# liangyuwang/Tiny-DeepSpeed

Measured on AMD Instinct MI355X. Metric: tokens/sec (whole node) GPT-2 ZeRO-2, higher is better.
Workload: dtype bf16; 1 GPU; model=gpt2-medium, global_batch=32, seq_len=1024, parallelism=zero2-dp1

## Files before the change

csrc/bind.cpp:

```cpp
#include <torch/extension.h>
#include <ATen/cuda/CUDAContext.h>

#include <hip/hip_runtime_api.h>

#include <array>
#include <cstring>
#include <vector>

extern "C" {
hipError_t tdsa_ln_fwd(const void*, const void*, void*, const void*,
                       const void*, void*, float*, float*, int, int, float,
                       int, hipStream_t);
int tdsa_ln_bwd_dx_stripes(int M);
hipError_t tdsa_ln_bwd_dx(const void*, const void*, const void*, const void*,
                          const float*, const float*, void*, float*, float*,
                          int, int, int, hipStream_t);
hipError_t tdsa_ln_bwd_dwdb(const float*, const float*, float*, float*, int,
                            int, hipStream_t);
hipError_t tdsa_gelu_fwd(const void*, void*, long long, int, hipStream_t);
hipError_t tdsa_gelu_bwd(const void*, const void*, void*, long long, int,
                         hipStream_t);
hipError_t tdsa_column_sum(const void*, float*, void*, int, int, int,
                           hipStream_t);
hipError_t tdsa_embedding_fwd(const void*, const long long*, void*, long long,
                              int, int, hipStream_t);
hipError_t tdsa_embedding_bwd(const void*, const long long*, const long long*,
                              float*, float*, long long, int, long long, int,
                              hipStream_t);
hipError_t tdsa_ce_fwd(const void*, const long long*, float*, float*, int*,
                       long long, int, long long, int, hipStream_t);
hipError_t tdsa_ce_bwd(const void*, const long long*, const float*, void*,
                       long long, int, float, long long, int, hipStream_t);
hipError_t tdsa_adamw_step(void*, const void*, float*, float*, float*, float*,
                           int, int, float, float, float, float, float,
                           long long, long long, int, int, hipStream_t);
hipError_t tdsa_adamw_multi(const void*, long long, int, int, float, float,
                            float, float, float, long long, hipStream_t);
int tdsa_adamw_desc_size();
int tdsa_adamw_chunkref_size();
int tdsa_sgd_desc_size();
hipError_t tdsa_sgd_multi(const void*, long long, int, int, float, float,
                          float, float, int, int, int, hipStream_t);
hipError_t tdsa_sgd_step(void*, const void*, float*, float*, int, int, float,
                         float, float, float, int, int, int, long long, int,
                         int, hipStream_t);
hipError_t tdsa_attn_fwd(const void*, const void*, const void*, void*, float*,
                         long long, long long, int, float, const long long*,
                         const long long*, float, unsigned long long,
                         hipStream_t);
hipError_t tdsa_attn_bwd(const void*, const void*, const void*, const void*,
                         const float*, const void*, void*, void*, void*, float*,
                         long long, long long, int, float, const long long*,
                         const long long*, const long long*, float,
                         unsigned long long, hipStream_t);
int tdsa_gemm_tn_splits(long long M, int N, int K);
hipError_t tdsa_gemm_tn(const void*, const void*, float*, long long, int, int,
                        hipStream_t);
hipError_t tdsa_dbg_mfma(const void*, const void*, float*, int, hipStream_t);
hipError_t tdsa_dbg_mfma32(const void*, const void*, float*, hipStream_t);
hipError_t tdsa_dbg_stage(const void*, void*, int, hipStream_t);
hipError_t tdsa_dbg_tr16(const void*, float*, hipStream_t);
}

namespace {

void check_hip(hipError_t err, const char* what) {
  TORCH_CHECK(err == hipSuccess, what, ": ", hipGetErrorString(err));
}

int dtype_flag(const at::Tensor& t) {
  if (t.scalar_type() == at::kBFloat16) return 1;
  if (t.scalar_type() == at::kFloat) return 0;
  TORCH_CHECK(false, "expected float32 or bfloat16, got ", t.scalar_type());
  return -1;
}

hipStream_t cur_stream() {
  return (hipStream_t)at::cuda::getCurrentCUDAStream().stream();
}

#define CHECK_IN(t)                                                     \
  TORCH_CHECK((t).is_cuda(), #t " must be on GPU");                     \
  TORCH_CHECK((t).is_contiguous(), #t " must be contiguous")

std::vector<at::Tensor> layernorm_fwd(at::Tensor x, at::Tensor w, at::Tensor b,
                                      double eps,
                                      c10::optional<at::Tensor> res) {
  CHECK_IN(x); CHECK_IN(w); CHECK_IN(b);
  const int N = x.size(-1);
  const long long M = x.numel() / N;
  auto y = at::empty_like(x);
  auto f32 = x.options().dtype(at::kFloat);
  auto mean = at::empty({M}, f32);
  auto rstd = at::empty({M}, f32);
  at::Tensor h;
  void* res_p = nullptr;
  void* h_p = nullptr;
  if (res.has_value()) {
    CHECK_IN((*res));
    h = at::empty_like(x);
    res_p = res->data_ptr();
    h_p = h.data_ptr();
  }
  check_hip(tdsa_ln_fwd(x.data_ptr(), res_p, h_p, w.data_ptr(), b.data_ptr(),
                        y.data_ptr(), mean.data_ptr<float>(),
                        rstd.data_ptr<float>(), (int)M, N, (float)eps,
                        dtype_flag(x), cur_stream()),
            "layernorm_fwd");
  auto row_sizes = x.sizes().vec();
  row_sizes.pop_back();
  if (res.has_value())
    return {y, mean.view(row_sizes), rstd.view(row_sizes), h};
  return {y, mean.view(row_sizes), rstd.view(row_sizes)};
}

std::vector<at::Tensor> layernorm_bwd_dx(at::Tensor dy, at::Tensor x,
                                         at::Tensor w, at::Tensor mean,
                                         at::Tensor rstd, int64_t n_stripes,
                                         c10::optional<at::Tensor> dh) {
  CHECK_IN(dy); CHECK_IN(x); CHECK_IN(w);
  (void)n_stripes;
  const int N = x.size(-1);
  const long long M = x.numel() / N;
  const int G = tdsa_ln_bwd_dx_stripes((int)M);
  auto dx = at::empty_like(x);
  auto f32 = x.options().dtype(at::kFloat);
  auto pdw = at::empty({G, N}, f32);
  auto pdb = at::empty({G, N}, f32);
  auto meanc = mean.contiguous();
  auto rstdc = rstd.contiguous();
  at::Tensor dhc;
  void* dh_p = nullptr;
  if (dh.has_value()) {
    dhc = dh->contiguous();
    dh_p = dhc.data_ptr();
  }
  check_hip(tdsa_ln_bwd_dx(dy.data_ptr(), dh_p, x.data_ptr(), w.data_ptr(),
                           meanc.data_ptr<float>(), rstdc.data_ptr<float>(),
                           dx.data_ptr(), pdw.data_ptr<float>(),
                           pdb.data_ptr<float>(), (int)M, N, dtype_flag(x),
                           cur_stream()),
            "layernorm_bwd_dx");
  return {dx, pdw, pdb};
}

std::vector<at::Tensor> layernorm_bwd_dwdb(at::Tensor pdw, at::Tensor pdb) {
  CHECK_IN(pdw); CHECK_IN(pdb);
  const int G = pdw.size(0);
  const int N = pdw.size(1);
  auto dw = at::empty({N}, pdw.options());
  auto db = at::empty({N}, pdb.options());
  check_hip(tdsa_ln_bwd_dwdb(pdw.data_ptr<float>(), pdb.data_ptr<float>(),
                             dw.data_ptr<float>(), db.data_ptr<float>(), G, N,
                             cur_stream()),
            "layernorm_bwd_dwdb");
  return {dw, db};
}

at::Tensor gelu_fwd(at::Tensor x) {
  CHECK_IN(x);
  auto y = at::empty_like(x);
  check_hip(tdsa_gelu_fwd(x.data_ptr(), y.data_ptr(), x.numel(), dtype_flag(x),
                          cur_stream()),
            "gelu_fwd");
  return y;
}

at::Tensor gelu_bwd(at::Tensor dy, at::Tensor x) {
  CHECK_IN(dy); CHECK_IN(x);
  auto dx = at::empty_like(x);
  check_hip(tdsa_gelu_bwd(dy.data_ptr(), x.data_ptr(), dx.data_ptr(), x.numel(),
                          dtype_flag(x), cur_stream()),
            "gelu_bwd");
  return dx;
}

at::Tensor column_sum(at::Tensor dy) {
  CHECK_IN(dy);
  TORCH_CHECK(dy.dim() == 2, "column_sum expects 2-D input");
  const int M = dy.size(0);
  const int N = dy.size(1);
  auto out32 = at::zeros({N}, dy.options().dtype(at::kFloat));
  auto out = at::empty({N}, dy.options());
  check_hip(tdsa_column_sum(dy.data_ptr(), out32.data_ptr<float>(),
                            out.data_ptr(), M, N, dtype_flag(dy), cur_stream()),
            "column_sum");
  return out;
}

at::Tensor embedding_fwd(at::Tensor weight, at::Tensor idx) {
  CHECK_IN(weight); CHECK_IN(idx);
  TORCH_CHECK(idx.scalar_type() == at::kLong, "idx must be int64");
  const long long R = idx.numel();
  const int D = weight.size(1);
  auto out = at::empty({R, (long long)D}, weight.options());
  check_hip(tdsa_embedding_fwd(weight.data_ptr(), (const long long*)idx.data_ptr<int64_t>(),
                               out.data_ptr(), R, D, dtype_flag(weight),
                               cur_stream()),
            "embedding_fwd");
  return out;
}

at::Tensor embedding_bwd(at::Tensor dy, at::Tensor idx, int64_t num_embeddings,
                         int64_t padding_idx) {
  CHECK_IN(dy); CHECK_IN(idx);
  TORCH_CHECK(idx.scalar_type() == at::kLong, "idx must be int64");
  const long long R = idx.numel();
  const int D = dy.size(-1);
  auto dw32 = at::zeros({num_embeddings, (long long)D},
                        dy.options().dtype(at::kFloat));
  auto sorted = at::sort(idx.reshape({-1}), true, 0,
                         false);
  auto sidx = std::get<0>(sorted).contiguous();
  auto perm = std::get<1>(sorted).contiguous();
  auto part = at::empty({R, (long long)D}, dy.options().dtype(at::kFloat));
  check_hip(tdsa_embedding_bwd(dy.data_ptr(), (const long long*)sidx.data_ptr<int64_t>(),
                               (const long long*)perm.data_ptr<int64_t>(),
                               dw32.data_ptr<float>(), part.data_ptr<float>(),
                               R, D, padding_idx, dtype_flag(dy),
                               cur_stream()),
            "embedding_bwd");
  return dw32;
}

std::vector<at::Tensor> cross_entropy_fwd(at::Tensor logits, at::Tensor targets,
                                          int64_t ignore_index) {
  CHECK_IN(logits); CHECK_IN(targets);
  TORCH_CHECK(logits.dim() == 2, "logits must be 2-D");
  TORCH_CHECK(targets.scalar_type() == at::kLong, "targets must be int64");
  const long long R = logits.size(0);
  const int V = logits.size(1);
  auto f32 = logits.options().dtype(at::kFloat);
  auto lse = at::empty({R}, f32);
  auto row_loss = at::empty({R}, f32);
  auto n_valid32 = at::zeros({}, logits.options().dtype(at::kInt));
  check_hip(tdsa_ce_fwd(logits.data_ptr(), (const long long*)targets.data_ptr<int64_t>(),
                        lse.data_ptr<float>(), row_loss.data_ptr<float>(),
                        n_valid32.data_ptr<int>(), R, V, ignore_index,
                        dtype_flag(logits), cur_stream()),
            "cross_entropy_fwd");
  return {row_loss.sum(), lse, n_valid32.to(at::kLong)};
}

at::Tensor cross_entropy_bwd(at::Tensor logits, at::Tensor targets,
                             at::Tensor lse, double dloss, int64_t n_valid,
                             int64_t ignore_index,
                             c10::optional<at::Tensor> out) {
  CHECK_IN(logits); CHECK_IN(targets); CHECK_IN(lse);
  const long long R = logits.size(0);
  const int V = logits.size(1);
  at::Tensor dlogits;
  if (out.has_value()) {
    dlogits = *out;
    CHECK_IN(dlogits);
    TORCH_CHECK(dlogits.sizes() == logits.sizes()
                && dlogits.scalar_type() == logits.scalar_type(),
                "cross_entropy_bwd: out must match logits");
  } else {
    dlogits = at::empty_like(logits);
  }
  const float scale = (float)(dloss / (double)std::max<int64_t>(n_valid, 1));
  check_hip(tdsa_ce_bwd(logits.data_ptr(), (const long long*)targets.data_ptr<int64_t>(),
                        lse.data_ptr<float>(), dlogits.data_ptr(), R, V, scale,
                        ignore_index, dtype_flag(logits), cur_stream()),
            "cross_entropy_bwd");
  return dlogits;
}

void adamw_step(at::Tensor param, at::Tensor grad, at::Tensor m, at::Tensor v,
                at::Tensor master, at::Tensor vmax, bool has_master,
                bool amsgrad, double lr, double b1, double b2, double eps,
                double wd, int64_t step) {
  CHECK_IN(param); CHECK_IN(grad); CHECK_IN(m); CHECK_IN(v);
  check_hip(tdsa_adamw_step(param.data_ptr(), grad.data_ptr(),
                            m.data_ptr<float>(), v.data_ptr<float>(),
                            has_master ? master.data_ptr<float>() : nullptr,
                            amsgrad ? vmax.data_ptr<float>() : nullptr,
                            has_master, amsgrad, (float)lr, (float)b1,
                            (float)b2, (float)eps, (float)wd, step,
                            param.numel(), dtype_flag(param), dtype_flag(grad),
                            cur_stream()),
            "adamw_step");
}

void adamw_step_multi(std::vector<at::Tensor> params,
                      std::vector<at::Tensor> grads,
                      std::vector<at::Tensor> ms, std::vector<at::Tensor> vs,
                      std::vector<c10::optional<at::Tensor>> masters,
                      double lr, double b1, double b2, double eps, double wd,
                      int64_t step) {
  const size_t n = params.size();
  TORCH_CHECK(grads.size() == n && ms.size() == n && vs.size() == n &&
              masters.size() == n, "length mismatch");
  if (n == 0) return;
  struct Desc {
    void* p; const void* g; float* m; float* v; float* master;
    long long numel; int param_bf16; int grad_bf16;
  };
  struct CRef { int tensor; int chunk; };
  TORCH_CHECK((int)sizeof(Desc) == tdsa_adamw_desc_size());
  TORCH_CHECK((int)sizeof(CRef) == tdsa_adamw_chunkref_size());
  const int chunk_elems = 1 << 16;
  std::vector<Desc> descs(n);
  std::vector<CRef> chunks;
  chunks.reserve(1024);
  for (size_t i = 0; i < n; ++i) {
    auto& p = params[i];
    auto& g = grads[i];
    Desc d;
// ... 77 lines not shown
  check_hip(tdsa_sgd_step(param.data_ptr(), grad.data_ptr(),
                          has_buf ? buf.data_ptr<float>() : nullptr,
                          has_master ? master.data_ptr<float>() : nullptr,
                          has_buf, has_master, (float)lr, (float)momentum,
                          (float)dampening, (float)wd, nesterov, maximize,
                          first_step, param.numel(), dtype_flag(param),
                          dtype_flag(grad), cur_stream()),
            "sgd_step");
}

at::Tensor gemm_tn(at::Tensor dy2, at::Tensor x2) {
  CHECK_IN(dy2); CHECK_IN(x2);
  TORCH_CHECK(dy2.dim() == 2 && x2.dim() == 2, "gemm_tn expects 2-D inputs");
  TORCH_CHECK(dy2.scalar_type() == at::kBFloat16
              && x2.scalar_type() == at::kBFloat16, "gemm_tn is bf16-only");
  TORCH_CHECK(dy2.size(0) == x2.size(0), "reduction dims differ");
  const long long M = dy2.size(0);
  const int N = dy2.size(1);
  const int K = x2.size(1);
  const int splits = tdsa_gemm_tn_splits(M, N, K);
  TORCH_CHECK(splits > 0, "gemm_tn: unsupported shape (need M%64==0, "
              "N%128==0, K%128==0), got ", M, "x", N, "/", K);
  auto f32 = dy2.options().dtype(at::kFloat);
  auto dw32 = at::empty({(long long)splits, (long long)N, (long long)K}, f32);
  check_hip(tdsa_gemm_tn(dy2.data_ptr(), x2.data_ptr(),
                         dw32.data_ptr<float>(), M, N, K, cur_stream()),
            "gemm_tn");
  return (splits > 1 ? dw32.sum(0) : dw32.select(0, 0)).to(at::kBFloat16);
}

static void check_attn_tensor(const at::Tensor& t, const char* name) {
  TORCH_CHECK(t.is_cuda(), name, " must be on GPU");
  TORCH_CHECK(t.dim() == 4 && t.size(3) == 64, name,
              ": attention kernel requires (B,H,T,64)");
  TORCH_CHECK(t.scalar_type() == at::kBFloat16, name, " must be bf16");
  TORCH_CHECK(t.stride(3) == 1, name, " last dim must be contiguous");
}

static std::array<long long, 3> strides3(const at::Tensor& t) {
  return {(long long)t.stride(0), (long long)t.stride(1),
          (long long)t.stride(2)};
}

std::vector<at::Tensor> attention_fwd(at::Tensor q, at::Tensor k, at::Tensor v,
                                      double scale,
                                      c10::optional<at::Tensor> out,
                                      double dropout_p, int64_t seed) {
  check_attn_tensor(q, "q");
  check_attn_tensor(k, "k");
  check_attn_tensor(v, "v");
  TORCH_CHECK(q.strides() == k.strides() && q.strides() == v.strides(),
              "q/k/v must share strides");
  TORCH_CHECK(q.size(2) % 64 == 0, "attention kernel requires T %% 64 == 0");
  const long long B = q.size(0), H = q.size(1);
  const int T = q.size(2);
  at::Tensor o = out.has_value() ? *out : at::empty_like(q);
  check_attn_tensor(o, "o");
  auto lse = at::empty({B, H, (long long)T}, q.options().dtype(at::kFloat));
  auto sq = strides3(q);
  auto so = strides3(o);
  TORCH_CHECK(dropout_p >= 0.0 && dropout_p < 1.0, "bad dropout_p");
  check_hip(tdsa_attn_fwd(q.data_ptr(), k.data_ptr(), v.data_ptr(),
                          o.data_ptr(), lse.data_ptr<float>(), B, H, T,
                          (float)scale, sq.data(), so.data(), (float)dropout_p,
                          (unsigned long long)seed, cur_stream()),
            "attention_fwd");
  return {o, lse};
}

std::vector<at::Tensor> attention_bwd(at::Tensor q, at::Tensor k, at::Tensor v,
                                      at::Tensor o, at::Tensor lse,
                                      at::Tensor dout, double scale,
                                      c10::optional<at::Tensor> dq_out,
                                      c10::optional<at::Tensor> dk_out,
                                      c10::optional<at::Tensor> dv_out,
                                      double dropout_p, int64_t seed) {
  check_attn_tensor(q, "q");
  check_attn_tensor(k, "k");
  check_attn_tensor(v, "v");
  check_attn_tensor(o, "o");
  check_attn_tensor(dout, "dout");
  TORCH_CHECK(q.strides() == k.strides() && q.strides() == v.strides(),
              "q/k/v must share strides");
  TORCH_CHECK(o.strides() == dout.strides(), "o/dout must share strides");
  auto lsec = lse.contiguous();
  const long long B = q.size(0), H = q.size(1);
  const int T = q.size(2);
  at::Tensor dq = dq_out.has_value() ? *dq_out : at::empty_like(q);
  at::Tensor dk = dk_out.has_value() ? *dk_out : at::empty_like(k);
  at::Tensor dv = dv_out.has_value() ? *dv_out : at::empty_like(v);
  TORCH_CHECK(dq.strides() == dk.strides() && dq.strides() == dv.strides(),
              "dq/dk/dv must share strides");
  auto delta = at::empty({B * H * T}, q.options().dtype(at::kFloat));
  auto sq = strides3(q);
  auto so = strides3(o);
  auto sd = strides3(dq);
  check_hip(tdsa_attn_bwd(q.data_ptr(), k.data_ptr(), v.data_ptr(),
                          o.data_ptr(), lsec.data_ptr<float>(), dout.data_ptr(),
                          dq.data_ptr(), dk.data_ptr(), dv.data_ptr(),
                          delta.data_ptr<float>(), B, H, T, (float)scale,
                          sq.data(), so.data(), sd.data(), (float)dropout_p,
                          (unsigned long long)seed, cur_stream()),
            "attention_bwd");
  return {dq, dk, dv};
}

at::Tensor dbg_mfma(at::Tensor A, at::Tensor B, int64_t variant) {
  CHECK_IN(A); CHECK_IN(B);
  auto D = at::zeros({16, 16}, A.options().dtype(at::kFloat));
  check_hip(tdsa_dbg_mfma(A.data_ptr(), B.data_ptr(), D.data_ptr<float>(),
                          (int)variant, cur_stream()),
            "dbg_mfma");
  return D;
}

at::Tensor dbg_mfma32(at::Tensor A, at::Tensor B) {
  CHECK_IN(A); CHECK_IN(B);
  auto D = at::zeros({32, 32}, A.options().dtype(at::kFloat));
  check_hip(tdsa_dbg_mfma32(A.data_ptr(), B.data_ptr(), D.data_ptr<float>(),
                            cur_stream()),
            "dbg_mfma32");
  return D;
}

at::Tensor dbg_stage(at::Tensor in, int64_t transposed) {
  CHECK_IN(in);
  auto out = at::zeros_like(in);
  check_hip(tdsa_dbg_stage(in.data_ptr(), out.data_ptr(), (int)transposed,
                           cur_stream()),
            "dbg_stage");
  return out;
}

at::Tensor dbg_tr16(at::Tensor in) {
  CHECK_IN(in);
  auto out = at::zeros({2, 4, 2, 4, 64}, in.options().dtype(at::kFloat));
  check_hip(tdsa_dbg_tr16(in.data_ptr(), out.data_ptr<float>(), cur_stream()),
            "dbg_tr16");
  return out;
}

}

PYBIND11_MODULE(TORCH_EXTENSION_NAME, mod) {
  mod.def("dbg_mfma", &dbg_mfma);
  mod.def("dbg_mfma32", &dbg_mfma32);
  mod.def("dbg_stage", &dbg_stage);
  mod.def("dbg_tr16", &dbg_tr16);
  mod.def("layernorm_fwd", &layernorm_fwd, py::arg("x"), py::arg("w"),
          py::arg("b"), py::arg("eps"), py::arg("res") = py::none());
  mod.def("layernorm_bwd_dx", &layernorm_bwd_dx, py::arg("dy"), py::arg("x"),
          py::arg("w"), py::arg("mean"), py::arg("rstd"),
          py::arg("n_stripes"), py::arg("dh") = py::none());
  mod.def("layernorm_bwd_dwdb", &layernorm_bwd_dwdb);
  mod.def("gelu_fwd", &gelu_fwd);
  mod.def("gelu_bwd", &gelu_bwd);
  mod.def("column_sum", &column_sum);
  mod.def("embedding_fwd", &embedding_fwd);
  mod.def("embedding_bwd", &embedding_bwd);
  mod.def("cross_entropy_fwd", &cross_entropy_fwd);
  mod.def("cross_entropy_bwd", &cross_entropy_bwd, py::arg("logits"),
          py::arg("targets"), py::arg("lse"), py::arg("dloss"),
          py::arg("n_valid"), py::arg("ignore_index"),
          py::arg("out") = py::none());
  mod.def("gemm_tn", &gemm_tn);
  mod.def("adamw_step", &adamw_step);
  mod.def("adamw_step_multi", &adamw_step_multi);
  mod.def("sgd_step", &sgd_step);
  mod.def("sgd_step_multi", &sgd_step_multi);
  mod.def("attention_fwd", &attention_fwd, py::arg("q"), py::arg("k"),
          py::arg("v"), py::arg("scale"), py::arg("out") = py::none(),
          py::arg("dropout_p") = 0.0, py::arg("seed") = 0);
  mod.def("attention_bwd", &attention_bwd, py::arg("q"), py::arg("k"),
          py::arg("v"), py::arg("o"), py::arg("lse"), py::arg("dout"),
          py::arg("scale"), py::arg("dq") = py::none(),
          py::arg("dk") = py::none(), py::arg("dv") = py::none(),
          py::arg("dropout_p") = 0.0, py::arg("seed") = 0);
}
```

csrc/kernels/layernorm.hip:

```cpp
#include "common.h"

#include <cstdlib>

namespace tdsa {

template <typename T> struct VecTraits;
template <> struct VecTraits<float> {
  static constexpr int W = 4;
  typedef float4v V;
  static DEV_INLINE V load(const float* p) { return *reinterpret_cast<const V*>(p); }
  static DEV_INLINE float get(V v, int i) { return v[i]; }
  static DEV_INLINE void set(V& v, int i, float x) { v[i] = x; }
  static DEV_INLINE void store(float* p, V v) { *reinterpret_cast<V*>(p) = v; }
};
template <> struct VecTraits<bf16> {
  static constexpr int W = 8;
  typedef short8v V;
  static DEV_INLINE V load(const bf16* p) { return load8(p); }
  static DEV_INLINE float get(V v, int i) { return bf_elem(v, i); }
  static DEV_INLINE void set(V& v, int i, float x) { v[i] = bf_pack(x); }
  static DEV_INLINE void store(bf16* p, V v) { store8(p, v); }
};

template <typename T, bool HAS_RES, int MAXITER = 2, bool ONE_WAVE = false>
// ... 58 lines not shown
        typename VT::V ov;
#pragma unroll
        for (int k = 0; k < W; ++k) {
          float xh = (VT::get(xv, k) - mu) * rs;
          VT::set(ov, k, xh * VT::get(wv, k) + VT::get(bv, k));
        }
        VT::store(yr + i, ov);
      }
    }
  }
}

template <typename T, int MAXITER, bool HAS_DH, bool STRIPES = true,
          bool ONE_WAVE = false>
__global__ void ln_bwd_dx_kernel(const T* __restrict__ dy, const T* __restrict__ dh,
                                 const T* __restrict__ x,
                                 const T* __restrict__ w, const float* __restrict__ mean,
                                 const float* __restrict__ rstd, T* __restrict__ dx,
                                 float* __restrict__ pdw, float* __restrict__ pdb,
                                 int M, int N) {
  using VT = VecTraits<T>;
  constexpr int W = VT::W;
  __shared__ float scratch[2 * 1024 / WAVE];
  const int tid = threadIdx.x;
  const int nth = blockDim.x;
  float accdw[MAXITER][W];
  float accdb[MAXITER][W];
#pragma unroll
  for (int it = 0; it < MAXITER; ++it)
#pragma unroll
    for (int k = 0; k < W; ++k) accdw[it][k] = accdb[it][k] = 0.f;

  for (int row = blockIdx.x; row < M; row += gridDim.x) {
    const T* dyr = dy + (long long)row * N;
    const T* xr = x + (long long)row * N;
    const float mu = mean[row];
    const float rs = rstd[row];
    typename VT::V dyc[MAXITER], xc[MAXITER];
    float c1 = 0.f, c2 = 0.f;
    {
      int it = 0;
      for (int i = tid * W; i < N; i += nth * W, ++it) {
        typename VT::V dv = VT::load(dyr + i);
        typename VT::V xv = VT::load(xr + i);
        typename VT::V wv = VT::load(w + i);
        dyc[it] = dv;
        xc[it] = xv;
#pragma unroll
        for (int k = 0; k < W; ++k) {
          float d = VT::get(dv, k);
          float xh = (VT::get(xv, k) - mu) * rs;
          float wdy = VT::get(wv, k) * d;
          c1 += xh * wdy;
          c2 += wdy;
          if (STRIPES) {
            accdw[it][k] += d * xh;
            accdb[it][k] += d;
          }
        }
      }
    }
    if (ONE_WAVE) {
      c1 = wave_sum(c1);
      c2 = wave_sum(c2);
    } else {
      block_sum2(c1, c2, scratch);
    }
    c1 /= N;
    c2 /= N;
    T* dxr = dx + (long long)row * N;
    const T* dhr = HAS_DH ? dh + (long long)row * N : nullptr;
    {
      int it = 0;
      for (int i = tid * W; i < N; i += nth * W, ++it) {
        typename VT::V dv = dyc[it];
        typename VT::V xv = xc[it];
        typename VT::V wv = VT::load(w + i);
        typename VT::V hv;
        if (HAS_DH) hv = VT::load(dhr + i);
        typename VT::V ov;
#pragma unroll
        for (int k = 0; k < W; ++k) {
          float d = VT::get(dv, k);
          float xh = (VT::get(xv, k) - mu) * rs;
          float wdy = VT::get(wv, k) * d;
          float g = (wdy - (xh * c1 + c2)) * rs;
          if (HAS_DH) g += VT::get(hv, k);
          VT::set(ov, k, g);
        }
        VT::store(dxr + i, ov);
      }
    }
  }
  if (STRIPES) {
    float* sdw = pdw + (long long)blockIdx.x * N;
    float* sdb = pdb + (long long)blockIdx.x * N;
    int it = 0;
    for (int i = tid * W; i < N; i += nth * W, ++it) {
#pragma unroll
      for (int k = 0; k < W; ++k) {
        sdw[i + k] = accdw[it][k];
        sdb[i + k] = accdb[it][k];
      }
    }
  }
}

template <typename T, int MAXITER>
__global__ void ln_dwdb_accum_kernel(const T* __restrict__ dy,
                                     const T* __restrict__ x,
                                     const float* __restrict__ mean,
                                     const float* __restrict__ rstd,
                                     float* __restrict__ pdw,
                                     float* __restrict__ pdb, int M, int N) {
  using VT = VecTraits<T>;
  constexpr int W = VT::W;
  const int tid = threadIdx.x;
  const int nth = blockDim.x;
  float accdw[MAXITER][W];
  float accdb[MAXITER][W];
#pragma unroll
  for (int it = 0; it < MAXITER; ++it)
#pragma unroll
    for (int k = 0; k < W; ++k) accdw[it][k] = accdb[it][k] = 0.f;
  for (int row = blockIdx.x; row < M; row += gridDim.x) {
    const T* dyr = dy + (long long)row * N;
    const T* xr = x + (long long)row * N;
    const float mu = mean[row];
    const float rs = rstd[row];
    int it = 0;
    for (int i = tid * W; i < N; i += nth * W, ++it) {
      typename VT::V dv = VT::load(dyr + i);
      typename VT::V xv = VT::load(xr + i);
#pragma unroll
      for (int k = 0; k < W; ++k) {
        float d = VT::get(dv, k);
        accdw[it][k] += d * (VT::get(xv, k) - mu) * rs;
        accdb[it][k] += d;
      }
    }
  }
  float* sdw = pdw + (long long)blockIdx.x * N;
  float* sdb = pdb + (long long)blockIdx.x * N;
  int it = 0;
  for (int i = tid * W; i < N; i += nth * W, ++it) {
#pragma unroll
    for (int k = 0; k < W; ++k) {
      sdw[i + k] = accdw[it][k];
      sdb[i + k] = accdb[it][k];
    }
  }
}

template <typename T, bool HAS_RES>
__global__ void ln_fwd_wide_kernel(const T* __restrict__ x,
                                   const T* __restrict__ res, T* __restrict__ h,
                                   const T* __restrict__ w, const T* __restrict__ b,
                                   T* __restrict__ y, float* __restrict__ mean,
                                   float* __restrict__ rstd, int M, int N,
                                   float eps) {
  using VT = VecTraits<T>;
  constexpr int W = VT::W;
  __shared__ float scratch[2 * 1024 / WAVE];
  const int tid = threadIdx.x;
  const int nth = blockDim.x;
  for (int row = blockIdx.x; row < M; row += gridDim.x) {
    const T* xr = x + (long long)row * N;
    const T* rr = HAS_RES ? res + (long long)row * N : nullptr;
    T* hr = HAS_RES ? h + (long long)row * N : nullptr;
    float s = 0.f, ss = 0.f;
    for (int i = tid * W; i < N; i += nth * W) {
      typename VT::V v = VT::load(xr + i);
      if (HAS_RES) {
        typename VT::V rv = VT::load(rr + i);
        typename VT::V hv;
#pragma unroll
        for (int k = 0; k < W; ++k)
          VT::set(hv, k, VT::get(v, k) + VT::get(rv, k));
        VT::store(hr + i, hv);
        v = hv;
      }
#pragma unroll
      for (int k = 0; k < W; ++k) {
        float f = VT::get(v, k);
        s += f;
        ss += f * f;
      }
    }
    block_sum2(s, ss, scratch);
    const float mu = s / N;
    const float var = fmaxf(ss / N - mu * mu, 0.0f);
    const float rs = rsqrtf(var + eps);
    if (tid == 0) {
      mean[row] = mu;
      rstd[row] = rs;
    }
    const T* src = HAS_RES ? hr : xr;
    T* yr = y + (long long)row * N;
    for (int i = tid * W; i < N; i += nth * W) {
      typename VT::V xv = VT::load(src + i);
      typename VT::V wv = VT::load(w + i);
      typename VT::V bv = VT::load(b + i);
      typename VT::V ov;
#pragma unroll
      for (int k = 0; k < W; ++k) {
        float xh = (VT::get(xv, k) - mu) * rs;
        VT::set(ov, k, xh * VT::get(wv, k) + VT::get(bv, k));
      }
      VT::store(yr + i, ov);
    }
  }
}

template <typename T, bool HAS_DH>
__global__ void ln_bwd_dx_wide_kernel(const T* __restrict__ dy,
                                      const T* __restrict__ dh,
                                      const T* __restrict__ x,
                                      const T* __restrict__ w,
                                      const float* __restrict__ mean,
                                      const float* __restrict__ rstd,
                                      T* __restrict__ dx, float* __restrict__ pdw,
                                      float* __restrict__ pdb, int M, int N) {
  using VT = VecTraits<T>;
  constexpr int W = VT::W;
  __shared__ float scratch[2 * 1024 / WAVE];
  const int tid = threadIdx.x;
  const int nth = blockDim.x;
  float* sdw = pdw + (long long)blockIdx.x * N;
  float* sdb = pdb + (long long)blockIdx.x * N;
  for (int i = tid; i < N; i += nth) {
    sdw[i] = 0.f;
    sdb[i] = 0.f;
  }
  for (int row = blockIdx.x; row < M; row += gridDim.x) {
    const T* dyr = dy + (long long)row * N;
    const T* xr = x + (long long)row * N;
    const float mu = mean[row];
    const float rs = rstd[row];
    float c1 = 0.f, c2 = 0.f;
    for (int i = tid * W; i < N; i += nth * W) {
      typename VT::V dv = VT::load(dyr + i);
      typename VT::V xv = VT::load(xr + i);
      typename VT::V wv = VT::load(w + i);
#pragma unroll
      for (int k = 0; k < W; ++k) {
        float d = VT::get(dv, k);
        float xh = (VT::get(xv, k) - mu) * rs;
        float wdy = VT::get(wv, k) * d;
        c1 += xh * wdy;
        c2 += wdy;
      }
    }
    block_sum2(c1, c2, scratch);
    c1 /= N;
    c2 /= N;
    T* dxr = dx + (long long)row * N;
    const T* dhr = HAS_DH ? dh + (long long)row * N : nullptr;
    for (int i = tid * W; i < N; i += nth * W) {
      typename VT::V dv = VT::load(dyr + i);
      typename VT::V xv = VT::load(xr + i);
      typename VT::V wv = VT::load(w + i);
      typename VT::V hv;
      if (HAS_DH) hv = VT::load(dhr + i);
      typename VT::V ov;
#pragma unroll
      for (int k = 0; k < W; ++k) {
        float d = VT::get(dv, k);
        float xh = (VT::get(xv, k) - mu) * rs;
        float wdy = VT::get(wv, k) * d;
        float g = (wdy - (xh * c1 + c2)) * rs;
        if (HAS_DH) g += VT::get(hv, k);
        VT::set(ov, k, g);
        sdw[i + k] += d * xh;
        sdb[i + k] += d;
      }
      VT::store(dxr + i, ov);
    }
  }
}

__global__ void ln_bwd_dwdb_kernel(const float* __restrict__ pdw,
                                   const float* __restrict__ pdb,
                                   float* __restrict__ dw, float* __restrict__ db,
                                   int G, int N) {
  const int c = blockIdx.x * (blockDim.x / WAVE) + threadIdx.x / WAVE;
  if (c >= N) return;
  const int lane = threadIdx.x & (WAVE - 1);
  float sw = 0.f, sb = 0.f;
  for (int g = lane; g < G; g += WAVE) {
    sw += pdw[(long long)g * N + c];
    sb += pdb[(long long)g * N + c];
  }
  sw = wave_sum(sw);
  sb = wave_sum(sb);
  if (lane == 0) {
    dw[c] = sw;
    db[c] = sb;
  }
}

}

using namespace tdsa;

extern "C" {

static int ln_block(int N, int W) {
  int need = (N + W - 1) / W;
  int blk = ((need + 63) / 64) * 64;
  if (blk > 256) blk = 256;
  if (blk < 64) blk = 64;
  return blk;
}

hipError_t tdsa_ln_fwd(const void* x, const void* res, void* h, const void* w,
                       const void* b, void* y, float* mean, float* rstd,
                       int M, int N, float eps, int is_bf16,
                       hipStream_t stream) {
  const int block = ln_block(N, is_bf16 ? 8 : 4);
  int cap = 32768;
  if (const char* v = getenv("TDSA_LN_GRID")) cap = atoi(v);
  const int grid = (M < cap) ? M : cap;
  int wave_ok = 0;
  if (const char* v = getenv("TDSA_LN_WAVE")) wave_ok = atoi(v);
#define LN_FWD(T, HASR)                                                       \
  hipLaunchKernelGGL((ln_fwd_kernel<T, HASR>), dim3(grid), dim3(block), 0,    \
                     stream, (const T*)x, (const T*)res, (T*)h, (const T*)w,  \
                     (const T*)b, (T*)y, mean, rstd, M, N, eps)
#define LN_FWD_OW(T, HASR)                                                    \
  hipLaunchKernelGGL((ln_fwd_kernel<T, HASR, 4, true>), dim3(grid),           \
                     dim3(WAVE), 0, stream, (const T*)x, (const T*)res,       \
                     (T*)h, (const T*)w, (const T*)b, (T*)y, mean, rstd, M,   \
                     N, eps)
#define LN_FWD_WIDE(T, HASR)                                                  \
  hipLaunchKernelGGL((ln_fwd_wide_kernel<T, HASR>), dim3(grid), dim3(1024),   \
                     0, stream, (const T*)x, (const T*)res, (T*)h,            \
                     (const T*)w, (const T*)b, (T*)y, mean, rstd, M, N, eps)
  if (is_bf16) {
    if (N % 8) return hipErrorInvalidValue;
    if (wave_ok && N <= 4 * WAVE * 8) {
      if (res) LN_FWD_OW(bf16, true); else LN_FWD_OW(bf16, false);
    } else if (N > 2 * block * 8) {
      if (res) LN_FWD_WIDE(bf16, true); else LN_FWD_WIDE(bf16, false);
    } else {
      if (res) LN_FWD(bf16, true); else LN_FWD(bf16, false);
    }
  } else {
    if (N % 4) return hipErrorInvalidValue;
    if (wave_ok && N <= 4 * WAVE * 4) {
      if (res) LN_FWD_OW(float, true); else LN_FWD_OW(float, false);
    } else if (N > 2 * block * 4) {
      if (res) LN_FWD_WIDE(float, true); else LN_FWD_WIDE(float, false);
    } else {
      if (res) LN_FWD(float, true); else LN_FWD(float, false);
    }
  }
#undef LN_FWD
#undef LN_FWD_OW
#undef LN_FWD_WIDE
  return hipGetLastError();
}

int tdsa_ln_bwd_dx_stripes(int M) {
  int cap = 2048;
  if (const char* v = getenv("TDSA_LN_STRIPES")) cap = atoi(v);
  int g = M < cap ? M : cap;
  return g < 1 ? 1 : g;
}

hipError_t tdsa_ln_bwd_dx(const void* dy, const void* dh, const void* x,
                          const void* w, const float* mean, const float* rstd,
                          void* dx, float* pdw, float* pdb, int M, int N,
                          int is_bf16, hipStream_t stream) {
  const int block = ln_block(N, is_bf16 ? 8 : 4);
  const int grid = tdsa_ln_bwd_dx_stripes(M);
  int split = 1;
  if (const char* v = getenv("TDSA_LN_SPLIT")) split = atoi(v);
  int dx_cap = 32768;
  if (const char* v = getenv("TDSA_LN_GRID")) dx_cap = atoi(v);
  const int dx_grid = split ? ((M < dx_cap) ? M : dx_cap) : grid;
  int wave_ok = 0;
  if (const char* v = getenv("TDSA_LN_WAVE")) wave_ok = atoi(v);
  const int ow = wave_ok && N <= 4 * WAVE * (is_bf16 ? 8 : 4);
#define LN_BWD(T, HASD)                                                        \
  do {                                                                         \
    if (split && ow) {                                                         \
      hipLaunchKernelGGL((ln_bwd_dx_kernel<T, 4, HASD, false, true>),          \
                         dim3(dx_grid), dim3(WAVE), 0, stream, (const T*)dy,   \
                         (const T*)dh, (const T*)x, (const T*)w, mean, rstd,   \
                         (T*)dx, pdw, pdb, M, N);                              \
      hipLaunchKernelGGL((ln_dwdb_accum_kernel<T, 2>), dim3(grid),             \
                         dim3(block), 0, stream, (const T*)dy, (const T*)x,    \
                         mean, rstd, pdw, pdb, M, N);                          \
    } else if (split) {                                                        \
      hipLaunchKernelGGL((ln_bwd_dx_kernel<T, 2, HASD, false>), dim3(dx_grid), \
                         dim3(block), 0, stream, (const T*)dy, (const T*)dh,   \
                         (const T*)x, (const T*)w, mean, rstd, (T*)dx, pdw,    \
                         pdb, M, N);                                           \
      hipLaunchKernelGGL((ln_dwdb_accum_kernel<T, 2>), dim3(grid),             \
                         dim3(block), 0, stream, (const T*)dy, (const T*)x,    \
                         mean, rstd, pdw, pdb, M, N);                          \
    } else {                                                                   \
      hipLaunchKernelGGL((ln_bwd_dx_kernel<T, 2, HASD, true>), dim3(grid),     \
                         dim3(block), 0, stream, (const T*)dy, (const T*)dh,   \
                         (const T*)x, (const T*)w, mean, rstd, (T*)dx, pdw,    \
                         pdb, M, N);                                           \
    }                                                                          \
  } while (0)
#define LN_BWD_WIDE(T, HASD)                                                  \
  hipLaunchKernelGGL((ln_bwd_dx_wide_kernel<T, HASD>), dim3(grid),            \
                     dim3(1024), 0, stream, (const T*)dy, (const T*)dh,       \
                     (const T*)x, (const T*)w, mean, rstd, (T*)dx, pdw, pdb,  \
                     M, N)
  if (is_bf16) {
    if (N % 8) return hipErrorInvalidValue;
    if (N > 2 * block * 8) {
      if (dh) LN_BWD_WIDE(bf16, true); else LN_BWD_WIDE(bf16, false);
    } else {
      if (dh) LN_BWD(bf16, true); else LN_BWD(bf16, false);
    }
  } else {
    if (N % 4) return hipErrorInvalidValue;
    if (N > 2 * block * 4) {
      if (dh) LN_BWD_WIDE(float, true); else LN_BWD_WIDE(float, false);
    } else {
      if (dh) LN_BWD(float, true); else LN_BWD(float, false);
    }
  }
#undef LN_BWD
#undef LN_BWD_WIDE
  return hipGetLastError();
}

hipError_t tdsa_ln_bwd_dwdb(const float* pdw, const float* pdb, float* dw,
                            float* db, int G, int N, hipStream_t stream) {
  const int block = 256;
  const int cols_per_block = block / WAVE;
  const int grid = (N + cols_per_block - 1) / cols_per_block;
  hipLaunchKernelGGL(ln_bwd_dwdb_kernel, dim3(grid), dim3(block), 0, stream,
                     pdw, pdb, dw, db, G, N);
  return hipGetLastError();
}

}
```

tiny_deepspeed_amd/ops/layernorm.py:

```python

import torch

from . import _ext
from .autotuner import default_tuner

N_STRIPES = 256


def ln_fwd_hip(x, weight, bias, eps):
    return _ext.get_ext().layernorm_fwd(x.contiguous(), weight, bias, eps)


def ln_fwd_torch(x, weight, bias, eps):
    xf = x.float()
    mean = xf.mean(dim=-1)
    var = xf.var(dim=-1, unbiased=False)
    rstd = (var + eps).rsqrt()
    y = (xf - mean.unsqueeze(-1)) * rstd.unsqueeze(-1)
    y = y * weight.float() + bias.float()
    return y.to(x.dtype), mean, rstd


def layernorm_fwd(x, weight, bias, eps=1e-5, tuner=None):
    if not _ext.use_native(x):
        return ln_fwd_torch(x, weight, bias, eps)
    tuner = tuner if tuner is not None else default_tuner()
    if tuner is not None:
        return tuner.choose("ln_fwd", [ln_fwd_hip, ln_fwd_torch],
                            x, weight, bias, eps)
    return ln_fwd_hip(x, weight, bias, eps)


def ln_fwd_res_hip(x, res, weight, bias, eps):
    y, mean, rstd, h = _ext.get_ext().layernorm_fwd(
        x.contiguous(), weight, bias, eps, res.contiguous()
    )
    return h, y, mean, rstd


def ln_fwd_res_torch(x, res, weight, bias, eps):
    h = x + res
    y, mean, rstd = ln_fwd_torch(h, weight, bias, eps)
    return h, y, mean, rstd


def layernorm_fwd_res(x, res, weight, bias, eps=1e-5, tuner=None):
    if not _ext.use_native(x):
        return ln_fwd_res_torch(x, res, weight, bias, eps)
    tuner = tuner if tuner is not None else default_tuner()
    if tuner is not None:
        return tuner.choose("ln_fwd_res", [ln_fwd_res_hip, ln_fwd_res_torch],
                            x, res, weight, bias, eps)
    return ln_fwd_res_hip(x, res, weight, bias, eps)


def ln_dx_hip(dy, x, weight, mean, rstd, dh):
    dx, pdw, pdb = _ext.get_ext().layernorm_bwd_dx(
        dy.contiguous(), x.contiguous(), weight, mean, rstd, N_STRIPES, dh
    )
    return dx, (pdw, pdb)


def ln_dx_torch(dy, x, weight, mean, rstd, dh):
    xf = x.float()
    dyf = dy.float()
    wf = weight.float()
    xhat = (xf - mean.unsqueeze(-1)) * rstd.unsqueeze(-1)
    wdy = wf * dyf
    c1 = (xhat * wdy).mean(dim=-1, keepdim=True)
    c2 = wdy.mean(dim=-1, keepdim=True)
    dx = (wdy - (xhat * c1 + c2)) * rstd.unsqueeze(-1)
    if dh is not None:
        dx = dx + dh.float()
    return dx.to(x.dtype), (dy, x, mean, rstd)


def layernorm_dx(dy, x, weight, mean, rstd, dh=None, tuner=None):
    if not _ext.use_native(dy):
        return ln_dx_torch(dy, x, weight, mean, rstd, dh)
    tuner = tuner if tuner is not None else default_tuner()
    if tuner is not None:
        return tuner.choose("ln_dx", [ln_dx_hip, ln_dx_torch],
                            dy, x, weight, mean, rstd, dh)
    return ln_dx_hip(dy, x, weight, mean, rstd, dh)


def layernorm_dwdb(workspace, dtype=None, tuner=None):
    if len(workspace) == 2:
        pdw, pdb = workspace
        if _ext.use_native(pdw):
            ext = _ext.get_ext()
            dw, db = ext.layernorm_bwd_dwdb(pdw, pdb)
            if dtype is not None:
                dw, db = dw.to(dtype), db.to(dtype)
            return dw, db
        dw = pdw.sum(dim=0)
        db = pdb.sum(dim=0)
    else:
        dy, x, mean, rstd = workspace
        xf = x.float().reshape(-1, x.shape[-1])
        dyf = dy.float().reshape(-1, dy.shape[-1])
        xhat = (xf - mean.reshape(-1, 1)) * rstd.reshape(-1, 1)
        dw = (dyf * xhat).sum(dim=0)
        db = dyf.sum(dim=0)
    if dtype is not None:
        dw, db = dw.to(dtype), db.to(dtype)
    return dw, db
```

Measured before the change: 307,300 tokens/s.

## Add one-wave-per-row LayerNorm kernels and a shared-memory dW/dB reduction with bf16 output

Adds row-per-wavefront LayerNorm forward and backward kernels for bf16 with N up to 2048. Weights and bias stay in registers, several rows are prefetched per iteration, and reductions use wave shuffles only, with no block-level syncs. The backward pass keeps per-wave dW/dB partials in registers and writes one stripe per wave. The dW/dB finalize kernel is rewritten as a 1024-thread column-slab reduction through shared memory that can emit bf16 directly, which removes a separate cast kernel. The costs are higher register pressure and more partial stripes (up to 2048 waves) for the final reduction to sum.

Result: faster. 325,800 tokens/s (median of 6 runs) (+6.0%).

```diff
diff --git a/csrc/bind.cpp b/csrc/bind.cpp
--- a/csrc/bind.cpp
+++ b/csrc/bind.cpp
@@ -11,11 +11,12 @@
 hipError_t tdsa_ln_fwd(const void*, const void*, void*, const void*,
                        const void*, void*, float*, float*, int, int, float,
                        int, hipStream_t);
-int tdsa_ln_bwd_dx_stripes(int M);
+int tdsa_ln_bwd_dx_stripes(int M, int N, int is_bf16);
+void tdsa_ln_rowwave_info(int, int, int, int*, int*, int*, int*);
 hipError_t tdsa_ln_bwd_dx(const void*, const void*, const void*, const void*,
                           const float*, const float*, void*, float*, float*,
                           int, int, int, hipStream_t);
-hipError_t tdsa_ln_bwd_dwdb(const float*, const float*, float*, float*, int,
+hipError_t tdsa_ln_bwd_dwdb(const float*, const float*, void*, void*, int, int,
                             int, hipStream_t);
 hipError_t tdsa_gelu_fwd(const void*, void*, long long, int, hipStream_t);
 hipError_t tdsa_gelu_bwd(const void*, const void*, void*, long long, int,
@@ -122,7 +123,7 @@
   (void)n_stripes;
   const int N = x.size(-1);
   const long long M = x.numel() / N;
-  const int G = tdsa_ln_bwd_dx_stripes((int)M);
+  const int G = tdsa_ln_bwd_dx_stripes((int)M, N, dtype_flag(x));
   auto dx = at::empty_like(x);
   auto f32 = x.options().dtype(at::kFloat);
   auto pdw = at::empty({G, N}, f32);
@@ -144,17 +145,28 @@
   return {dx, pdw, pdb};
 }
 
-std::vector<at::Tensor> layernorm_bwd_dwdb(at::Tensor pdw, at::Tensor pdb) {
+std::vector<at::Tensor> layernorm_bwd_dwdb(
+    at::Tensor pdw, at::Tensor pdb, c10::optional<at::ScalarType> dtype) {
   CHECK_IN(pdw); CHECK_IN(pdb);
+  const at::ScalarType out = dtype.value_or(at::kFloat);
+  TORCH_CHECK(out == at::kFloat || out == at::kBFloat16,
+              "layernorm_bwd_dwdb: dtype must be float32 or bfloat16");
   const int G = pdw.size(0);
   const int N = pdw.size(1);
-  auto dw = at::empty({N}, pdw.options());
-  auto db = at::empty({N}, pdb.options());
+  auto dw = at::empty({N}, pdw.options().dtype(out));
+  auto db = at::empty({N}, pdb.options().dtype(out));
   check_hip(tdsa_ln_bwd_dwdb(pdw.data_ptr<float>(), pdb.data_ptr<float>(),
-                             dw.data_ptr<float>(), db.data_ptr<float>(), G, N,
-                             cur_stream()),
+                             dw.data_ptr(), db.data_ptr(), G, N,
+                             out == at::kBFloat16, cur_stream()),
             "layernorm_bwd_dwdb");
   return {dw, db};
+}
+
+std::vector<int64_t> layernorm_rowwave_geometry(int64_t M, int64_t N,
+                                                bool is_bf16) {
+  int fw = 0, fd = 0, bd = 0, bound = 0;
+  tdsa_ln_rowwave_info((int)M, (int)N, is_bf16, &fw, &fd, &bd, &bound);
+  return {tdsa_ln_bwd_dx_stripes((int)M, (int)N, is_bf16), fw, fd, bd, bound};
 }
 
 at::Tensor gelu_fwd(at::Tensor x) {
@@ -538,7 +550,10 @@
   mod.def("layernorm_bwd_dx", &layernorm_bwd_dx, py::arg("dy"), py::arg("x"),
           py::arg("w"), py::arg("mean"), py::arg("rstd"),
           py::arg("n_stripes"), py::arg("dh") = py::none());
-  mod.def("layernorm_bwd_dwdb", &layernorm_bwd_dwdb);
+  mod.def("layernorm_bwd_dwdb", &layernorm_bwd_dwdb, py::arg("pdw"),
+          py::arg("pdb"), py::arg("dtype") = py::none());
+  mod.def("layernorm_rowwave_geometry", &layernorm_rowwave_geometry,
+          py::arg("M"), py::arg("N"), py::arg("is_bf16") = true);
   mod.def("gelu_fwd", &gelu_fwd);
   mod.def("gelu_bwd", &gelu_bwd);
   mod.def("column_sum", &column_sum);
diff --git a/csrc/kernels/layernorm.hip b/csrc/kernels/layernorm.hip
--- a/csrc/kernels/layernorm.hip
+++ b/csrc/kernels/layernorm.hip
@@ -234,6 +234,239 @@
   }
 }
 
+#define LN_RW_BLOCK 256
+#define LN_RW_WAVES (LN_RW_BLOCK / WAVE)
+#define LN_RW_MAXVEC 4
+#ifndef LN_RW_FWD_DEPTH
+#define LN_RW_FWD_DEPTH(NVEC) ((NVEC) <= 2 ? 4 : 2)
+#endif
+#ifndef LN_RW_BWD_DEPTH
+#define LN_RW_BWD_DEPTH(NVEC) 2
+#endif
+
+template <int NVEC>
+DEV_INLINE float ln_rw_row_sum(float (&p)[NVEC]) {
+#pragma unroll
+  for (int j = 0; j < NVEC; ++j) p[j] = wave_sum(p[j]);
+  if (NVEC == 1) return p[0];
+  if (NVEC == 2) return p[0] + p[1];
+  if (NVEC == 3) return (p[0] + p[2]) + p[1];
+  return (p[0] + p[2]) + (p[1] + p[NVEC - 1]);
+}
+
+template <typename T, bool HAS_RES, int NVEC, int R>
+__global__ __launch_bounds__(LN_RW_BLOCK) void ln_fwd_rowwave_kernel(
+    const T* __restrict__ x, const T* __restrict__ res, T* __restrict__ h,
+    const T* __restrict__ w, const T* __restrict__ b, T* __restrict__ y,
+    float* __restrict__ mean, float* __restrict__ rstd, int M, int N,
+    float eps) {
+  using VT = VecTraits<T>;
+  typedef typename VT::V V;
+  constexpr int W = VT::W;
+  const int lane = threadIdx.x & (WAVE - 1);
+  const int g = __builtin_amdgcn_readfirstlane(
+      (int)(blockIdx.x * LN_RW_WAVES + threadIdx.x / WAVE));
+  const long long G = (long long)gridDim.x * LN_RW_WAVES;
+  const bool last_ok = (lane + (NVEC - 1) * WAVE) * W < N;
+  const unsigned voff = lane * W;
+  const V zero = {};
+  V wv[NVEC], bv[NVEC];
+#pragma unroll
+  for (int j = 0; j < NVEC; ++j) {
+    wv[j] = bv[j] = zero;
+    if (j < NVEC - 1 || last_ok) {
+      wv[j] = VT::load(w + voff + j * WAVE * W);
+      bv[j] = VT::load(b + voff + j * WAVE * W);
+    }
+  }
+  for (long long row0 = g; row0 < M; row0 += G * R) {
+    V xc[R][NVEC], rc[R][NVEC];
+#pragma unroll
+    for (int r = 0; r < R; ++r) {
+      const long long row = row0 + r * G;
+#pragma unroll
+      for (int j = 0; j < NVEC; ++j) xc[r][j] = rc[r][j] = zero;
+      if (row < M) {
+        const T* xr = x + row * N;
+        const T* rr = HAS_RES ? res + row * N : nullptr;
+#pragma unroll
+        for (int j = 0; j < NVEC; ++j) {
+          if (j < NVEC - 1 || last_ok) {
+            xc[r][j] = VT::load(xr + voff + j * WAVE * W);
+            if (HAS_RES) rc[r][j] = VT::load(rr + voff + j * WAVE * W);
+          }
+        }
+      }
+    }
+#pragma unroll
+    for (int r = 0; r < R; ++r) {
+      const long long row = row0 + r * G;
+      if (row < M) {
+        float ps[NVEC], pss[NVEC];
+#pragma unroll
+        for (int j = 0; j < NVEC; ++j) {
+          ps[j] = pss[j] = 0.f;
+          V v = xc[r][j];
+          if (HAS_RES) {
+            V hv;
+#pragma unroll
+            for (int k = 0; k < W; ++k)
+              VT::set(hv, k, VT::get(v, k) + VT::get(rc[r][j], k));
+            if (j < NVEC - 1 || last_ok)
+              VT::store(h + row * N + voff + j * WAVE * W, hv);
+            v = hv;
+            xc[r][j] = hv;
+          }
+#pragma unroll
+          for (int k = 0; k < W; ++k) {
+            float f = VT::get(v, k);
+            ps[j] += f;
+            pss[j] += f * f;
+          }
+        }
+        const float s = ln_rw_row_sum<NVEC>(ps);
+        const float ss = ln_rw_row_sum<NVEC>(pss);
+        const float mu = s / N;
+        const float var = fmaxf(ss / N - mu * mu, 0.0f);
+        const float rs = rsqrtf(var + eps);
+        if (lane == 0) {
+          mean[row] = mu;
+          rstd[row] = rs;
+        }
+#pragma unroll
+        for (int j = 0; j < NVEC; ++j) {
+          V ov;
+#pragma unroll
+          for (int k = 0; k < W; ++k) {
+            float xh = (VT::get(xc[r][j], k) - mu) * rs;
+            VT::set(ov, k, xh * VT::get(wv[j], k) + VT::get(bv[j], k));
+          }
+          if (j < NVEC - 1 || last_ok)
+            VT::store(y + row * N + voff + j * WAVE * W, ov);
+        }
+      }
+    }
+  }
+}
+
+template <typename T, bool HAS_DH, int NVEC, int R>
+__global__ __launch_bounds__(LN_RW_BLOCK) void ln_bwd_rowwave_kernel(
+    const T* __restrict__ dy, const T* __restrict__ dh, const T* __restrict__ x,
+    const T* __restrict__ w, const float* __restrict__ mean,
+    const float* __restrict__ rstd, T* __restrict__ dx,
+    float* __restrict__ pdw, float* __restrict__ pdb, int M, int N) {
+  using VT = VecTraits<T>;
+  typedef typename VT::V V;
+  constexpr int W = VT::W;
+  const int lane = threadIdx.x & (WAVE - 1);
+  const int g = __builtin_amdgcn_readfirstlane(
+      (int)(blockIdx.x * LN_RW_WAVES + threadIdx.x / WAVE));
+  const long long G = (long long)gridDim.x * LN_RW_WAVES;
+  const bool last_ok = (lane + (NVEC - 1) * WAVE) * W < N;
+  const unsigned voff = lane * W;
+  const V zero = {};
+  V wv[NVEC];
+  float accdw[NVEC][W], accdb[NVEC][W];
+#pragma unroll
+  for (int j = 0; j < NVEC; ++j) {
+    wv[j] = zero;
+    if (j < NVEC - 1 || last_ok) wv[j] = VT::load(w + voff + j * WAVE * W);
+#pragma unroll
+    for (int k = 0; k < W; ++k) accdw[j][k] = accdb[j][k] = 0.f;
+  }
+  for (long long row0 = g; row0 < M; row0 += G * R) {
+    V dyc[R][NVEC], xc[R][NVEC];
+    float mu[R], rs[R];
+#pragma unroll
+    for (int r = 0; r < R; ++r) {
+      const long long row = row0 + r * G;
+      mu[r] = rs[r] = 0.f;
+#pragma unroll
+      for (int j = 0; j < NVEC; ++j) dyc[r][j] = xc[r][j] = zero;
+      if (row < M) {
+        mu[r] = mean[row];
+        rs[r] = rstd[row];
+#pragma unroll
+        for (int j = 0; j < NVEC; ++j) {
+          if (j < NVEC - 1 || last_ok) {
+            dyc[r][j] = VT::load(dy + row * N + voff + j * WAVE * W);
+            xc[r][j] = VT::load(x + row * N + voff + j * WAVE * W);
+          }
+        }
+      }
+    }
+#pragma unroll
+    for (int r = 0; r < R; ++r) {
+      const long long row = row0 + r * G;
+      if (row < M) {
+        float p1[NVEC], p2[NVEC];
+#pragma unroll
+        for (int j = 0; j < NVEC; ++j) {
+          p1[j] = p2[j] = 0.f;
+          if (j < NVEC - 1 || last_ok) {
+#pragma unroll
+            for (int k = 0; k < W; ++k) {
+              float d = VT::get(dyc[r][j], k);
+              float xh = (VT::get(xc[r][j], k) - mu[r]) * rs[r];
+              float wdy = VT::get(wv[j], k) * d;
+              p1[j] += xh * wdy;
+              p2[j] += wdy;
+              accdw[j][k] += d * (VT::get(xc[r][j], k) - mu[r]) * rs[r];
+              accdb[j][k] += d;
+            }
+          }
+        }
+#pragma unroll
+        for (int j = 0; j < NVEC; ++j)
+          asm volatile("" : "+v"(dyc[r][j]), "+v"(xc[r][j]));
+        V hc[NVEC];
+        if (HAS_DH) {
+#pragma unroll
+          for (int j = 0; j < NVEC; ++j) {
+            hc[j] = zero;
+            if (j < NVEC - 1 || last_ok)
+              hc[j] = VT::load(dh + row * N + voff + j * WAVE * W);
+          }
+        }
+        const float c1 = ln_rw_row_sum<NVEC>(p1) / N;
+        const float c2 = ln_rw_row_sum<NVEC>(p2) / N;
+#pragma unroll
+        for (int j = 0; j < NVEC; ++j) {
+          V ov;
+#pragma unroll
+          for (int k = 0; k < W; ++k) {
+            float d = VT::get(dyc[r][j], k);
+            float xh = (VT::get(xc[r][j], k) - mu[r]) * rs[r];
+            float wdy = VT::get(wv[j], k) * d;
+            float gx = (wdy - (xh * c1 + c2)) * rs[r];
+            if (HAS_DH) gx += VT::get(hc[j], k);
+            VT::set(ov, k, gx);
+          }
+          if (j < NVEC - 1 || last_ok)
+            VT::store(dx + row * N + voff + j * WAVE * W, ov);
+        }
+      }
+    }
+  }
+  float* sdw = pdw + (long long)g * N;
+  float* sdb = pdb + (long long)g * N;
+#pragma unroll
+  for (int j = 0; j < NVEC; ++j) {
+    if (j < NVEC - 1 || last_ok) {
+      const unsigned col = voff + j * WAVE * W;
+#pragma unroll
+      for (int k = 0; k < W; k += 4) {
+        float4v vw = {accdw[j][k], accdw[j][k + 1], accdw[j][k + 2],
+                      accdw[j][k + 3]};
+        float4v vb = {accdb[j][k], accdb[j][k + 1], accdb[j][k + 2],
+                      accdb[j][k + 3]};
+        *reinterpret_cast<float4v*>(sdw + col + k) = vw;
+        *reinterpret_cast<float4v*>(sdb + col + k) = vb;
+      }
+    }
+  }
+}
+
 template <typename T, bool HAS_RES>
 __global__ void ln_fwd_wide_kernel(const T* __restrict__ x,
                                    const T* __restrict__ res, T* __restrict__ h,
@@ -361,23 +594,46 @@
   }
 }
 
-__global__ void ln_bwd_dwdb_kernel(const float* __restrict__ pdw,
-                                   const float* __restrict__ pdb,
-                                   float* __restrict__ dw, float* __restrict__ db,
-                                   int G, int N) {
-  const int c = blockIdx.x * (blockDim.x / WAVE) + threadIdx.x / WAVE;
-  if (c >= N) return;
-  const int lane = threadIdx.x & (WAVE - 1);
-  float sw = 0.f, sb = 0.f;
-  for (int g = lane; g < G; g += WAVE) {
-    sw += pdw[(long long)g * N + c];
-    sb += pdb[(long long)g * N + c];
-  }
-  sw = wave_sum(sw);
-  sb = wave_sum(sb);
-  if (lane == 0) {
-    dw[c] = sw;
-    db[c] = sb;
+#define LN_DWDB_BLOCK 1024
+#define LN_DWDB_SLAB 32
+#define LN_DWDB_SUB (LN_DWDB_BLOCK / LN_DWDB_SLAB)
+static_assert(LN_DWDB_SUB == WAVE / 2, "tree below assumes 64 partials");
+DEV_INLINE void ln_store_out(float* p, float v) { *p = v; }
+DEV_INLINE void ln_store_out(bf16* p, float v) { *p = f2bf(v); }
+
+template <typename OutT>
+__global__ __launch_bounds__(LN_DWDB_BLOCK) void ln_bwd_dwdb_kernel(
+    const float* __restrict__ pdw, const float* __restrict__ pdb,
+    OutT* __restrict__ dw, OutT* __restrict__ db, int G, int N) {
+  __shared__ float red[2][LN_DWDB_SUB][LN_DWDB_SLAB];
+  const int c = threadIdx.x % LN_DWDB_SLAB;
+  const int sub = threadIdx.x / LN_DWDB_SLAB;
+  const int col = blockIdx.x * LN_DWDB_SLAB + c;
+  float swa = 0.f, swb = 0.f, sba = 0.f, sbb = 0.f;
+  if (col < N) {
+#pragma unroll 4
+    for (int g = sub; g < G; g += WAVE) {
+      swa += pdw[(long long)g * N + col];
+      sba += pdb[(long long)g * N + col];
+      if (g + LN_DWDB_SUB < G) {
+        swb += pdw[(long long)(g + LN_DWDB_SUB) * N + col];
+        sbb += pdb[(long long)(g + LN_DWDB_SUB) * N + col];
+      }
+    }
+  }
+  red[0][sub][c] = swa + swb;
+  red[1][sub][c] = sba + sbb;
+#pragma unroll
+  for (int off = LN_DWDB_SUB / 2; off > 0; off >>= 1) {
+    __syncthreads();
+    if (sub < off) {
+      red[0][sub][c] += red[0][sub + off][c];
+      red[1][sub][c] += red[1][sub + off][c];
+    }
+  }
+  if (sub == 0 && col < N) {
+    ln_store_out(dw + col, red[0][0][c]);
+    ln_store_out(db + col, red[1][0][c]);
   }
 }
 
@@ -386,6 +642,37 @@
 using namespace tdsa;
 
 extern "C" {
+
+static int ln_rw_nvec(int N, int is_bf16) {
+  int on = 1;
+  if (const char* v = getenv("TDSA_LN_ROWWAVE")) on = atoi(v);
+  if (!on || !is_bf16 || N < 8 || N % 8) return 0;
+  const int nvec = (N / 8 + WAVE - 1) / WAVE;
+  return nvec <= LN_RW_MAXVEC ? nvec : 0;
+}
+
+static int ln_rw_waves(int M, int cap) {
+  long long g = ((long long)(M < 1 ? 1 : M) + LN_RW_WAVES - 1) / LN_RW_WAVES *
+                LN_RW_WAVES;
+  cap = cap / LN_RW_WAVES * LN_RW_WAVES;
+  if (cap < LN_RW_WAVES) cap = LN_RW_WAVES;
+  return (int)(g < cap ? g : cap);
+}
+
+static int ln_rw_fwd_waves(int M) {
+  int cap = 4096;
+  if (const char* v = getenv("TDSA_LN_RW_WAVES")) cap = atoi(v);
+  return ln_rw_waves(M, cap);
+}
+
+void tdsa_ln_rowwave_info(int M, int N, int is_bf16, int* fwd_waves,
+                          int* fwd_depth, int* bwd_depth, int* bound) {
+  const int nvec = ln_rw_nvec(N, is_bf16);
+  *fwd_waves = nvec ? ln_rw_fwd_waves(M) : 0;
+  *fwd_depth = nvec ? LN_RW_FWD_DEPTH(nvec) : 0;
+  *bwd_depth = nvec ? LN_RW_BWD_DEPTH(nvec) : 0;
+  *bound = LN_RW_MAXVEC * WAVE * 8;
+}
 
 static int ln_block(int N, int W) {
   int need = (N + W - 1) / W;
@@ -399,6 +686,28 @@
                        const void* b, void* y, float* mean, float* rstd,
                        int M, int N, float eps, int is_bf16,
                        hipStream_t stream) {
+  if (const int nvec = ln_rw_nvec(N, is_bf16)) {
+    const int grid = ln_rw_fwd_waves(M) / LN_RW_WAVES;
+#define LN_RW_FWD(HASR, NV)                                                   \
+  hipLaunchKernelGGL(                                                         \
+      (ln_fwd_rowwave_kernel<bf16, HASR, NV, LN_RW_FWD_DEPTH(NV)>),           \
+      dim3(grid), dim3(LN_RW_BLOCK), 0, stream, (const bf16*)x,               \
+      (const bf16*)res, (bf16*)h, (const bf16*)w, (const bf16*)b, (bf16*)y,   \
+      mean, rstd, M, N, eps)
+#define LN_RW_FWD_NV(NV)                                                      \
+  do {                                                                        \
+    if (res) LN_RW_FWD(true, NV); else LN_RW_FWD(false, NV);                  \
+  } while (0)
+    switch (nvec) {
+      case 1: LN_RW_FWD_NV(1); break;
+      case 2: LN_RW_FWD_NV(2); break;
+      case 3: LN_RW_FWD_NV(3); break;
+      default: LN_RW_FWD_NV(4); break;
+    }
+#undef LN_RW_FWD_NV
+#undef LN_RW_FWD
+    return hipGetLastError();
+  }
   const int block = ln_block(N, is_bf16 ? 8 : 4);
   int cap = 32768;
   if (const char* v = getenv("TDSA_LN_GRID")) cap = atoi(v);
@@ -443,9 +752,10 @@
   return hipGetLastError();
 }
 
-int tdsa_ln_bwd_dx_stripes(int M) {
+int tdsa_ln_bwd_dx_stripes(int M, int N, int is_bf16) {
   int cap = 2048;
   if (const char* v = getenv("TDSA_LN_STRIPES")) cap = atoi(v);
+  if (ln_rw_nvec(N, is_bf16)) return ln_rw_waves(M, cap);
   int g = M < cap ? M : cap;
   return g < 1 ? 1 : g;
 }
@@ -454,8 +764,30 @@
                           const void* w, const float* mean, const float* rstd,
                           void* dx, float* pdw, float* pdb, int M, int N,
                           int is_bf16, hipStream_t stream) {
+  if (const int nvec = ln_rw_nvec(N, is_bf16)) {
+    const int grid = tdsa_ln_bwd_dx_stripes(M, N, is_bf16) / LN_RW_WAVES;
+#define LN_RW_BWD(HASD, NV)                                                   \
+  hipLaunchKernelGGL(                                                         \
+      (ln_bwd_rowwave_kernel<bf16, HASD, NV, LN_RW_BWD_DEPTH(NV)>),           \
+      dim3(grid), dim3(LN_RW_BLOCK), 0, stream, (const bf16*)dy,              \
+      (const bf16*)dh, (const bf16*)x, (const bf16*)w, mean, rstd, (bf16*)dx, \
+      pdw, pdb, M, N)
+#define LN_RW_BWD_NV(NV)                                                      \
+  do {                                                                        \
+    if (dh) LN_RW_BWD(true, NV); else LN_RW_BWD(false, NV);                   \
+  } while (0)
+    switch (nvec) {
+      case 1: LN_RW_BWD_NV(1); break;
+      case 2: LN_RW_BWD_NV(2); break;
+      case 3: LN_RW_BWD_NV(3); break;
+      default: LN_RW_BWD_NV(4); break;
+    }
+#undef LN_RW_BWD_NV
+#undef LN_RW_BWD
+    return hipGetLastError();
+  }
   const int block = ln_block(N, is_bf16 ? 8 : 4);
-  const int grid = tdsa_ln_bwd_dx_stripes(M);
+  const int grid = tdsa_ln_bwd_dx_stripes(M, N, is_bf16);
   int split = 1;
   if (const char* v = getenv("TDSA_LN_SPLIT")) split = atoi(v);
   int dx_cap = 32768;
@@ -514,13 +846,18 @@
   return hipGetLastError();
 }
 
-hipError_t tdsa_ln_bwd_dwdb(const float* pdw, const float* pdb, float* dw,
-                            float* db, int G, int N, hipStream_t stream) {
-  const int block = 256;
-  const int cols_per_block = block / WAVE;
-  const int grid = (N + cols_per_block - 1) / cols_per_block;
-  hipLaunchKernelGGL(ln_bwd_dwdb_kernel, dim3(grid), dim3(block), 0, stream,
-                     pdw, pdb, dw, db, G, N);
+hipError_t tdsa_ln_bwd_dwdb(const float* pdw, const float* pdb, void* dw,
+                            void* db, int G, int N, int out_bf16,
+                            hipStream_t stream) {
+  const int grid = (N + LN_DWDB_SLAB - 1) / LN_DWDB_SLAB;
+  if (out_bf16)
+    hipLaunchKernelGGL(ln_bwd_dwdb_kernel<bf16>, dim3(grid),
+                       dim3(LN_DWDB_BLOCK), 0, stream, pdw, pdb, (bf16*)dw,
+                       (bf16*)db, G, N);
+  else
+    hipLaunchKernelGGL(ln_bwd_dwdb_kernel<float>, dim3(grid),
+                       dim3(LN_DWDB_BLOCK), 0, stream, pdw, pdb, (float*)dw,
+                       (float*)db, G, N);
   return hipGetLastError();
 }
 
diff --git a/tiny_deepspeed_amd/ops/layernorm.py b/tiny_deepspeed_amd/ops/layernorm.py
--- a/tiny_deepspeed_amd/ops/layernorm.py
+++ b/tiny_deepspeed_amd/ops/layernorm.py
@@ -90,10 +90,11 @@
         pdw, pdb = workspace
         if _ext.use_native(pdw):
             ext = _ext.get_ext()
+            if dtype in (None, torch.float32, torch.bfloat16):
+                dw, db = ext.layernorm_bwd_dwdb(pdw, pdb, dtype)
+                return dw, db
             dw, db = ext.layernorm_bwd_dwdb(pdw, pdb)
-            if dtype is not None:
-                dw, db = dw.to(dtype), db.to(dtype)
-            return dw, db
+            return dw.to(dtype), db.to(dtype)
         dw = pdw.sum(dim=0)
         db = pdb.sum(dim=0)
     else:
```
